# arthurlirui/IRON

Hardware: AMD Instinct MI355X
Metric: Mrays/s sphere-trace+GGX shade, drv/dragon 800x800 (synthetic S0) (higher is better)
Workload: dtype f32

## Files before the change

include/iron_hip.h:

```cpp
#ifndef IRON_HIP_H
#define IRON_HIP_H

#include <stddef.h>
#include <stdint.h>

#ifdef __cplusplus
extern "C" {
#endif

#define IRON_ABI_VERSION 1

typedef enum iron_status {
    IRON_OK = 0,
    IRON_ERR_BAD_ARG = -1,
    IRON_ERR_UNSUPPORTED = -2,
    IRON_ERR_HIP = -3,
    IRON_ERR_NO_DEVICE = -4,
    IRON_ERR_WORKSPACE = -5,
    IRON_ERR_RANGE = -6
} iron_status;

int iron_version(void);
const char* iron_strerror(int status);
int iron_last_hip_error(void);
// ... 245 lines not shown
                     const float* ray_d, const float* in0, const float* in1, const float* in2, const float* in3, const uint8_t* work,
                     int64_t n, uint8_t* mask_out, uint8_t* unfinished_out, float* points, float* sdf_out, float* dist,
                     void* workspace, size_t workspace_bytes, void* stream);

int iron_trace_phase(int32_t phase, const iron_net_t* sdf, const iron_trace_params* p, const float* lin_steps,
                     const float* ray_o, const float* ray_d, const float* near, const float* far,
                     const uint8_t* work, const int64_t* ray_index, int64_t n, int32_t* chunk_iters,
                     int64_t n_chunks, uint8_t* conv, float* points, float* sdf_out, float* dist,
                     iron_trace_stats* stats, void* workspace, size_t workspace_bytes, void* stream);

typedef struct iron_shade_nets {
    const iron_net_t* sdf;
    const iron_net_t* diffuse_albedo;
    const iron_net_t* specular_albedo;
    const iron_net_t* specular_roughness;
} iron_shade_nets;

typedef struct iron_shade_out {
    float* color;
    float* diffuse_color;
    float* specular_color;
    float* diffuse_albedo;
    float* specular_albedo;
    float* specular_roughness;
    float* normal;
} iron_shade_out;

size_t iron_shade_workspace_bytes(int64_t n);

int iron_shade_ggx(const iron_shade_nets* nets, float light, int32_t is_metal, const float* tab_trans,
                   const float* tab_diff_trans, const float* ray_o, const float* ray_d, const float* points,
                   const uint8_t* conv, int64_t n, const iron_shade_out* out, void* workspace,
                   size_t workspace_bytes, void* stream);

typedef struct iron_shade_comp_nets {
    const iron_net_t* sdf;
    const iron_net_t* diffuse_albedo;
    const iron_net_t* specular_albedo;
    const iron_net_t* specular_roughness;
    const iron_net_t* metallic;
    const iron_net_t* dielectric;
    const iron_net_t* metallic_eta;
    const iron_net_t* metallic_k;
    const iron_net_t* dielectric_eta;
} iron_shade_comp_nets;

typedef struct iron_shade_comp_out {
    float* color;
    float* diffuse_color;
    float* specular_color;
    float* diffuse_albedo;
    float* specular_albedo;
    float* specular_roughness;
    float* metallic_eta;
    float* metallic_k;
    float* dielectric_eta;
    float* normal;
    float* metallic_rgb;
    float* metallic;
    float* dielectric_rgb;
    float* dielectric;
} iron_shade_comp_out;

size_t iron_shade_composite_workspace_bytes(int64_t n);

int iron_shade_composite(const iron_shade_comp_nets* nets, float light, const float* tab_trans, const float* tab_diff_trans,
                         const float* ray_o, const float* ray_d, const float* points, const uint8_t* conv, int64_t n,
                         const iron_shade_comp_out* out, void* workspace, size_t workspace_bytes, void* stream);

int32_t iron_set_cu_limit(int32_t n_cus);

int32_t iron_set_trace_split(int32_t parts);

int iron_sdf_screen_forward(const iron_net_t* net, const float* x, int64_t n, float* out, void* stream);

int32_t iron_set_sampler_screen(int32_t on);
int iron_sampler_screen_debug(int32_t what, double value);
int iron_trace_screen_counts(const void* workspace, double* out, void* stream);

int32_t iron_set_sampler_stride(int32_t on);
int iron_trace_stride_counts(const void* workspace, double* out, void* stream);
int iron_trace_stride_detail(const void* workspace, double* out, void* stream);

enum {
    IRON_PROF_SPHERE = 0, IRON_PROF_SAMPLER = 1, IRON_PROF_BISECT_A = 2, IRON_PROF_BISECT_B = 3,
    IRON_PROF_SDF_GRAD = 4, IRON_PROF_MATERIAL = 5, IRON_PROF_GGX = 6, IRON_PROF_SDF_FORWARD = 7,
    IRON_PROF_KINDS = 8
};
int iron_profile_enable(int32_t on);
int iron_profile_read(double* ms, int64_t* launches);

#ifdef __cplusplus
}
#endif
#endif
```

iron_amd/_lib.py:

```python
from __future__ import annotations

import ctypes as C
import os
import threading
from typing import Optional

import torch

_HERE = os.path.dirname(os.path.abspath(__file__))
LIB_PATH = os.path.join(_HERE, "csrc", "libiron_hip.so")

IRON_OK = 0
IRON_NET_NERF = 2
IRON_ERR_UNSUPPORTED = -2
IRON_ERR_RANGE = -6
IRON_NET_SDF, IRON_NET_RENDER = 0, 1
MODES = {"idr": 0, "no_view_dir": 1, "no_normal": 2, "points_only": 3}


class IronError(RuntimeError):
    pass


class iron_linear(C.Structure):
# ... 83 lines not shown
    "iron_sdf_forward": (C.c_int, [_P, _P, _I64, _P, _I32, _P]),
    "iron_sdf_get_all_workspace_bytes": (_SZ, [_P, _I64]),
    "iron_sdf_get_all": (C.c_int, [_P, _P, _I64, _P, _P, _P, _P, _SZ, _P]),
    "iron_render_forward": (C.c_int, [_P, _P, _P, _P, _P, _I64, _P, _P]),
    "iron_camera_rays": (C.c_int, [C.POINTER(_F), C.POINTER(_F), _P, _I64, _P, _P, _P, _P]),
    "iron_intersect_sphere": (C.c_int, [_P, _P, _I64, _F, _P, _P, _P, _P]),
    "iron_ggx_colocated": (C.c_int, [_F, _P, _P, _P, _P, _P, _P, _P, _P, _I64, _P, _P, _P, _P]),
    "iron_composite_colocated": (C.c_int, [C.c_float, _P, _P, _P, _P, _P, _P, _I64, _P, _P, _P, _P, _P, _P]),
    "iron_coloc_head": (C.c_int, [_I32, C.c_float, C.c_float, C.c_float, _P, _P, _P, _P, _P, _P, _I64, _P, _P, _P, _P]),
    "iron_grid_points": (C.c_int, [_P, _P, _P, _I32, _I32, _I32, _P, _P]),
    "iron_mc_workspace_bytes": (C.c_int, [_I32, _I32, _I32, C.POINTER(_SZ)]),
    "iron_mc_count": (C.c_int, [_P, _I32, _I32, _I32, _F, _P, C.POINTER(_I64), C.POINTER(_I64), _P]),
    "iron_mc_emit": (C.c_int, [_P, _I32, _I32, _I32, _F, _P, _P, _P, _P]),
    "iron_bake_workspace_bytes": (C.c_int, [_I64, C.POINTER(_SZ)]),
    "iron_bake_count": (C.c_int, [_P, _I64, _P, _I64, _P, _I64, _I64, C.c_uint64, C.c_uint32, _P, _P, _P, C.POINTER(_I64), _P]),
    "iron_bake_sample": (C.c_int, [_P, _P, _P, _P, _I64, C.c_uint64, C.c_uint32, _P, _I64, _P, _P, _P, _P]),
    "iron_bake_sample_explicit": (C.c_int, [_P, _I64, _P, _P, _I64, _P, _I64, _P, _P, _P, _I64, _P, _P, _P]),
    "iron_bake_splat": (C.c_int, [_P, _P, _I32, _P, _I32, _I64, _I32, _I32, _I64, _P, _P, _P]),
    "iron_bake_resolve": (C.c_int, [_P, _I32, _I32, _I32, _P, _P, _P, _P]),
    "iron_bvh_workspace_bytes": (C.c_int, [_I64, C.POINTER(_SZ)]),
    "iron_bvh_keys": (C.c_int, [_P, _I64, _P, _I64, _P, _P, _P]),
    "iron_bvh_hierarchy": (C.c_int, [_P, _I64, _P, _P]),
    "iron_bvh_boxes": (C.c_int, [_P, _I64, _P, _I64, _P, _P, _P]),
    "iron_point_mesh_distance": (C.c_int, [_P, _I64, _P, _I64, _P, _P, _P, _P]),
    "iron_mesh_raycast": (C.c_int, [_P, _I64, _P, _P, _I64, _F, _F, _P, _P, _P, _P]),
    "iron_mesh_vertex_normals": (C.c_int, [_P, _I64, _P, _I64, _P, _P]),
    "iron_texture_fetch": (C.c_int, [_P, _P, _I32, _I32, _I32, _P, _I64, _I32, _P, _P, _P]),
    "iron_asset_shade_ggx": (C.c_int, [C.POINTER(iron_asset_mesh), _F, _P, _P, _P, _P, _P, _P, _P, _I64, C.POINTER(iron_asset_out), _P]),
    "iron_mesh_edge_keys": (C.c_int, [_P, _I64, _P, _I64, _P, _P, _P]),
    "iron_mesh_components": (C.c_int, [_P, _P, _I64, _P, _I64, _P, _P, _I32, C.POINTER(_I32), _P]),
    "iron_uv_workspace_bytes": (C.c_int, [_I64, C.POINTER(_SZ)]),
    "iron_uv_projections": (C.c_int, [_P, _I64, _P, _I64, _F, _F, _I32, _P, _P, _P, _P, _P, C.POINTER(_I32), C.POINTER(_I32), _P]),
    "iron_uv_project": (C.c_int, [_P, _P, _P, _I64, _P, _P, _P, _P]),
    "iron_uv_rotation_search": (C.c_int, [_P, _P, _I64, _I64, _P, _I32, _I32, _P, _P]),
    "iron_uv_apply": (C.c_int, [_P, _P, _I64, _P, _P, _F, _P, _P]),
    "iron_img_sqerr_workspace_bytes": (C.c_int, [_I64, C.POINTER(_SZ)]),
    "iron_img_sqerr": (C.c_int, [_P, _P, _I64, _I32, _P, _P, _P]),
    "iron_img_ssim_workspace_bytes": (C.c_int, [_I32, _I32, C.POINTER(_SZ)]),
    "iron_img_ssim": (C.c_int, [_P, _P, _I32, _I32, _I32, _P, _P, _P, _P]),
    "iron_lpips_prepare": (C.c_int, [_P, _P, _I32, _I32, _I32, _P, _P]),
    "iron_conv2d_relu": (C.c_int, [_P, _I32, _I32, _I32, _I32, _P, _P, _I32, _I32, _I32, _I32, _P, _P, _P]),
    "iron_maxpool3s2": (C.c_int, [_P, _I32, _I32, _I32, _I32, _P, _P]),
    "iron_lpips_tap": (C.c_int, [_P, _I32, _I32, _I32, _P, _P, _P]),
    "iron_lpips_workspace_bytes": (C.c_int, [_I32, _I32, C.POINTER(_SZ)]),
    "iron_lpips_forward": (C.c_int, [_P, _P, _I32, _I32, _I32, C.POINTER(iron_lpips_weights), _P, _P, _P]),
    "iron_neus_linspace": (C.c_int, [_P, _P, _P, _I64, _I32, _P, _P]),
    "iron_neus_outside_z": (C.c_int, [_P, _P, _I64, _I32, _F, _P, _P]),
    "iron_neus_points": (C.c_int, [_P, _P, _P, _I64, _I32, _P, _P]),
    "iron_neus_up_sample": (C.c_int, [_P, _P, _P, _P, _I64, _I32, _I32, _F, _P, _P]),
    "iron_neus_merge": (C.c_int, [_P, _P, _I32, _P, _P, _I32, _I64, _P, _P, _P]),
    "iron_neus_mid_points": (C.c_int, [_P, _P, _P, _I64, _I32, _F, _I32, _P, _P, _P, _P]),
    "iron_neus_need_background": (C.c_int, [_P, _I64, _I32, _I32, _P, _P]),
    "iron_neus_composite": (C.c_int, [C.POINTER(iron_neus_composite_args), _P]),
    "iron_neus_composite_alpha": (C.c_int, [C.POINTER(iron_neus_composite_args), _P, _P]),
    "iron_neus_outside_composite": (C.c_int, [_P, _P, _P, _P, _I64, _I32, _P, _P, _P, _P]),
    "iron_neus_sample_pdf": (C.c_int, [_P, _P, _P, _I64, _I32, _I32, _P, _P]),
    "iron_smith_g1": (C.c_int, [_P, _P, _I64, _P, _P]),
    "iron_nerf_forward": (C.c_int, [_P, _P, _P, _I64, _P, _P, _P]),
    "iron_edge_walk": (C.c_int, [_P, _P, _I64, _P, _I32, _F, _F, _P, _P, _P]),
    "iron_morph_closing3x3": (C.c_int, [_P, _I32, _I32, _P, _P, _P]),
    "iron_sobel_magnitude": (C.c_int, [_P, _I32, _I32, _P, _P]),
    "iron_edge_pixels": (C.c_int, [_P, _P, _I64, C.POINTER(_F), C.POINTER(_F), _I32, _I32, _P, _P, _P]),
    "iron_fill_holes": (C.c_int, [_P, _P, _P, _P, _I64, _P, _P, _P, _P, _P, _P]),
    "iron_edge_sides": (C.c_int, [_P, _P, C.POINTER(_F), _I64, _P, _P, _P]),
    "iron_edge_blend": (C.c_int, [_P, _P, _P, _P, _P, _P, _I64, _I64, _P, _P, _P, _P, _P]),
    "iron_trace_workspace_bytes": (_SZ, [_I64, C.POINTER(iron_trace_params)]),
    "iron_trace": (C.c_int, [_P, C.POINTER(iron_trace_params), _P, _P, _P, _P, _P, _P, _I64, _P, _P, _P, _P, _P,
                             _P, _SZ, _P]),
    "iron_trace_stage": (C.c_int, [_I32, _P, C.POINTER(iron_trace_params), _P, _P, _P, _P, _P, _P, _P, _P, _I64, _P, _P, _P, _P, _P,
                                   _P, _SZ, _P]),
    "iron_trace_phase": (C.c_int, [_I32, _P, C.POINTER(iron_trace_params), _P, _P, _P, _P, _P, _P, _P, _I64, _P,
                                   _I64, _P, _P, _P, _P, _P, _P, _SZ, _P]),
    "iron_net_numeric_status": (C.c_int, [_P, C.POINTER(C.c_int32), _P]),
    "iron_net_force_exact": (C.c_int, [_P, _I32]),
    "iron_set_cu_limit": (_I32, [_I32]),
    "iron_set_trace_split": (_I32, [_I32]),
    "iron_sdf_screen_forward": (C.c_int, [_P, _P, _I64, _P, _P]),
    "iron_set_sampler_screen": (_I32, [_I32]),
    "iron_sampler_screen_debug": (C.c_int, [_I32, C.c_double]),
    "iron_trace_screen_counts": (C.c_int, [_P, C.POINTER(C.c_double), _P]),
    "iron_set_sampler_stride": (_I32, [_I32]),
    "iron_trace_stride_counts": (C.c_int, [_P, C.POINTER(C.c_double), _P]),
    "iron_trace_stride_detail": (C.c_int, [_P, C.POINTER(C.c_double), _P]),
    "iron_profile_enable": (C.c_int, [_I32]),
    "iron_profile_read": (C.c_int, [C.POINTER(C.c_double), C.POINTER(_I64)]),
    "iron_shade_workspace_bytes": (_SZ, [_I64]),
    "iron_shade_composite_workspace_bytes": (_SZ, [_I64]),
    "iron_shade_composite": (C.c_int, [C.POINTER(iron_shade_comp_nets), _F, _P, _P, _P, _P, _P, _P, _I64,
                                       C.POINTER(iron_shade_comp_out), _P, _SZ, _P]),
    "iron_shade_ggx": (C.c_int, [C.POINTER(iron_shade_nets), _F, _I32, _P, _P, _P, _P, _P, _P, _I64,
                                 C.POINTER(iron_shade_out), _P, _SZ, _P]),
}

class iron_train_layer(C.Structure):
    _fields_ = [("weight_v", C.c_void_p), ("weight_g", C.c_void_p), ("bias", C.c_void_p), ("d_weight_v", C.c_void_p),
                ("d_weight_g", C.c_void_p), ("d_bias", C.c_void_p), ("out_dim", C.c_int32), ("in_dim", C.c_int32)]


class iron_sdf_train_desc(C.Structure):
    _fields_ = [("n_linear", C.c_int32), ("multires", C.c_int32), ("skip_layer", C.c_int32), ("layers", C.POINTER(iron_train_layer))]


class iron_render_train_desc(C.Structure):
    _fields_ = [("n_linear", C.c_int32), ("mode", C.c_int32), ("multires", C.c_int32), ("multires_view", C.c_int32),
                ("d_feature", C.c_int32), ("d_out", C.c_int32), ("skip_layer", C.c_int32), ("squeeze_out", C.c_int32),
                ("output_bias", C.c_float), ("output_scale", C.c_float), ("squeeze_out_scale", C.c_float),
                ("layers", C.POINTER(iron_train_layer))]


class iron_composite_grads_in(C.Structure):
    _fields_ = [(k, C.c_void_p) for k in ("d_rgb", "d_specular_rgb", "d_metallic_rgb", "d_dielectric_rgb", "d_env_light_out")]


class iron_composite_grads_out(C.Structure):
    _fields_ = [(k, C.c_void_p) for k in ("d_light", "d_distance", "d_normal", "d_viewdir", "d_diffuse_albedo", "d_specular_albedo",
                                          "d_specular_roughness", "d_metallic_eta", "d_metallic_k", "d_dielectric_eta", "d_env_light")]


class iron_nerf_train_desc(C.Structure):
    _fields_ = [("D", C.c_int32), ("W", C.c_int32), ("d_in", C.c_int32), ("d_in_view", C.c_int32), ("multires", C.c_int32),
                ("multires_view", C.c_int32), ("skip", C.c_int32), ("layers", C.POINTER(iron_train_layer))]


class iron_neus_composite_grads(C.Structure):
    _fields_ = [(k, C.c_void_p) for k in ("d_color", "d_weight_sum", "d_weights", "d_gradient_error", "relax_count", "d_sdf", "d_grad",
                                          "d_sample_color", "d_inv_s", "d_bg_density", "d_bg_color")]


TRAIN_LIB_PATH = os.path.join(os.path.dirname(LIB_PATH), "libiron_train.so")
TRAIN_SYMBOLS = {
    "iron_train_gemm_workspace_bytes": (_SZ, [_I32, _I32, _I32]),
    "iron_train_gemm": (C.c_int, [_I32, _I32, _I32, _I32, _I32, _P, _I32, _P, _I32, _F, _P, _I32, _P, _SZ, _P]),
    "iron_sdf_backward_workspace_bytes": (_SZ, [C.POINTER(iron_sdf_train_desc), _I64]),
    "iron_sdf_backward": (C.c_int, [C.POINTER(iron_sdf_train_desc), _P, _I64, _P, _P, _P, _P, _SZ, _P]),
    "iron_render_backward_workspace_bytes": (_SZ, [C.POINTER(iron_render_train_desc), _I64]),
    "iron_render_backward": (C.c_int, [C.POINTER(iron_render_train_desc), _P, _P, _P, _P, _I64, _P, _P, _P, _P, _P, _P, _SZ, _P]),
    "iron_ggx_colocated_backward": (C.c_int, [_F] + [_P] * 8 + [_I64] + [_P] * 10 + [_P]),
    "iron_composite_colocated_backward": (C.c_int, [_F, _P, _P, _P, C.POINTER(iron_composite_params), _P, _P, _I64,
                                                    C.POINTER(iron_composite_grads_in), C.POINTER(iron_composite_grads_out), _P]),
    "iron_coloc_head_backward": (C.c_int, [_I32, _F, _F, _F] + [_P] * 6 + [_I64] + [_P] * 10 + [_P]),
    "iron_nerf_backward_workspace_bytes": (_SZ, [C.POINTER(iron_nerf_train_desc), _I64]),
    "iron_nerf_backward": (C.c_int, [C.POINTER(iron_nerf_train_desc), _P, _P, _I64, _P, _P, _P, _SZ, _P]),
    "iron_neus_composite_backward": (C.c_int, [C.POINTER(iron_neus_composite_args), C.POINTER(iron_neus_composite_grads), _P]),
    "iron_train_last_hip_error": (C.c_int, []),
    "iron_train_last_blas_status": (C.c_int, []),
    "iron_train_numeric_status": (C.c_int, [_I32, _P]),
    "iron_pyramid_l2_workspace_bytes": (_SZ, [_I64, _I32, _I32]),
    "iron_pyramid_l2_forward": (C.c_int, [_P, _P, _I64, _I32, _I32, C.POINTER(C.c_float), _P, _P, _SZ, _P]),
    "iron_pyramid_l2_backward": (C.c_int, [_P, _P, _I64, _I32, _I32, C.POINTER(C.c_float), _P, _P, _SZ, _P, _P, _P]),
    "iron_ssim_workspace_bytes": (C.c_int, [_I32, _I32, _I32, _I32, _I32, _I32, C.POINTER(_SZ), C.POINTER(_SZ)]),
    "iron_ssim_forward": (C.c_int, [_P, _P, _I32, _I32, _I32, _I32, C.POINTER(C.c_float), _I32, C.c_double, C.c_double, _P, _I32, _P,
                                    _P, _SZ, _P]),
    "iron_ssim_backward": (C.c_int, [_P, _P, _I32, _I32, _I32, _I32, C.POINTER(C.c_float), _I32, C.c_double, C.c_double, _I32, _P, _P,
                                     _SZ, _P, _SZ, _P, _P, _P]),
    "iron_gaussian_filter": (C.c_int, [_P, _I64, _I32, _I32, C.POINTER(C.c_float), _I32, _P, _P]),
}

_lock = threading.Lock()
_lib: Optional[C.CDLL] = None
_train_lib: Optional[C.CDLL] = None


def load_train() -> C.CDLL:
    global _train_lib
    with _lock:
        if _train_lib is not None:
# ... 101 lines not shown
```

iron_amd/csrc/trace.hip:

```cpp
#include <atomic>
#include <mutex>
#include <stdlib.h>
#include "mlp_h2.h"
#include "ggx_core.h"
#include "h2_setup.h"

namespace iron {

constexpr int kMaxTraceSplits = 4;

#ifndef IRON_FAST_SOFTPLUS
#define IRON_FAST_SOFTPLUS 1
#endif
constexpr bool kFastActT = IRON_FAST_SOFTPLUS != 0;

struct SamplerQ {
    int n_list;
    int head;
    int n_cont;
    int n_done;
};

struct TraceCounters {
    int q_head;
// ... 80 lines not shown
constexpr int kResolvePerRay = 2;
constexpr uint8_t kRayPending = 2;
constexpr uint8_t kRayOverflowed = 1;
__device__ __forceinline__ float screen_delta(const ScreenWs& s) {
    return s.delta_override > 0.0f ? s.delta_override : fmaxf(kScreenK * __uint_as_float(*s.calib), kScreenFloor);
}

struct TraceWs {
    TraceCounters* cnt;
    int* sampler_list;
    int* root_list;
    float* root_lo;
    float* root_hi;
    float* root_flo;
    float* root_fhi;
    int* root_k;
    int* chunk_iters;
    int* chunk_roots;
    int n_chunks;
    unsigned long long* cont;
    int cont_cap;
    int ovf_pass;
    ScreenWs scr;
};

struct TraceArgs {
    const float* ray_o;
    const float* ray_d;
    const float* near;
    const float* far;
    const uint8_t* work;
    const int64_t* ray_index;
    const float* lin;
    uint8_t* conv;
    float* points;
    float* sdf;
    float* dist;
    int ray0;
    int n;
    int n_steps;
    int iters;
    float thr;
    long long chunk;
};

__device__ __forceinline__ int lane_rank(unsigned mask, int j) { return __popc(mask & ((1u << j) - 1u)); }
__device__ __forceinline__ int lane_rank64(unsigned long long mask, int j) { return __popcll(mask & ((1ull << j) - 1ull)); }

template <int HI = 32, int LO = 1, class T>
__device__ __forceinline__ T wave_sum(T x) {
#pragma unroll
    for (int off = HI; off >= LO; off >>= 1) x += __shfl_xor(x, off, 64);
    return x;
}
template <int HI = 32, int LO = 1>
__device__ __forceinline__ float wave_max(float x) {
#pragma unroll
    for (int off = HI; off >= LO; off >>= 1) x = fmaxf(x, __shfl_xor(x, off, 64));
    return x;
}

__device__ __forceinline__ void ray_origin_dir(const TraceArgs& a, int ray, float& ox, float& oy, float& oz, float& dx, float& dy, float& dz) {
    ox = a.ray_o[3 * (size_t)ray]; oy = a.ray_o[3 * (size_t)ray + 1]; oz = a.ray_o[3 * (size_t)ray + 2];
    dx = a.ray_d[3 * (size_t)ray]; dy = a.ray_d[3 * (size_t)ray + 1]; dz = a.ray_d[3 * (size_t)ray + 2];
}

struct BackendF32 {
    static constexpr int kThreads = 64;
    SdfNetDev net;
    WStream ws;
    int lane;
    __device__ __forceinline__ void init(const SdfNetDev& n, const H2StreamDev&, const H2Meta&) {
        net = n;
        lane = threadIdx.x;
        ws.init(net.blob, net.blob_bytes, lane);
    }
    __device__ __forceinline__ bool any(bool p) { return p; }
    __device__ __forceinline__ float eval(float x, float y, float z) { return sdf_eval<kFastActT>(net, ws, x, y, z, lane); }
    __device__ __forceinline__ void finish() {}
    __device__ __forceinline__ void park(int, float) {}
    __device__ __forceinline__ void park(int, int) {}
    __device__ __forceinline__ float unpark(int, float v) { return v; }
    __device__ __forceinline__ int unpark(int, int v) { return v; }
};

constexpr int kParkFields = 17;
constexpr int kLdsPark = kLdsH2Total;
constexpr int kLdsTraceTotal = kLdsPark + kParkFields * 256 * 4;
static_assert(kLdsTraceTotal <= 160 * 1024, "LDS of a tracer workgroup");

template <bool DEFER_TILES>
struct BackendH2T {
    static constexpr int kThreads = 256;
    Ring ring;
    char* lds;
    H2Meta m;
    int lane, wave, parity;
    __device__ __forceinline__ void init(const SdfNetDev&, const H2StreamDev& s, const H2Meta& meta) {
        extern __shared__ __attribute__((aligned(16))) char smem[];
        lds = smem;
        m = meta;
        lane = threadIdx.x & 63;
        wave = __builtin_amdgcn_readfirstlane(threadIdx.x >> 6);
        parity = 0;
        h2_setup(s, lds, ring);
    }
    __device__ __forceinline__ bool any(bool p) {
        volatile int* f = reinterpret_cast<volatile int*>(lds + kLdsMisc) + parity * 4;
        if (lane == 0) f[wave] = p ? 1 : 0;
        __syncthreads();
        const int r = f[0] | f[1] | f[2] | f[3];
        parity ^= 1;
        return r != 0;
    }
    __device__ __forceinline__ float eval(float x, float y, float z) {
        f32x16 hf[kHidTiles];
        sdf_hidden_stack_h2<kFastActT, DEFER_TILES>(ring, lds, m.n_hidden_layers, m.skip_layer, m.scale, x, y, z, lane, hf);
        return (row_dot_lds(lds + kLdsRows, hf, lane >> 5) + m.b_last) / m.scale;
    }
    template <int NP>
    __device__ __forceinline__ float eval_screen(float x, float y, float z) {
        return sdf_screen_value<kFastActT, NP>(ring, lds, m.n_hidden_layers, m.skip_layer, m.scale, m.b_last, x, y, z, lane);
    }
    __device__ __forceinline__ void finish() { ring.drain(); }
    __device__ __forceinline__ void park(int i, float v) { reinterpret_cast<float*>(lds + kLdsPark)[i * 256 + threadIdx.x] = v; }
    __device__ __forceinline__ void park(int i, int v) { reinterpret_cast<int*>(lds + kLdsPark)[i * 256 + threadIdx.x] = v; }
    __device__ __forceinline__ float unpark(int i, float) { return reinterpret_cast<const float*>(lds + kLdsPark)[i * 256 + threadIdx.x]; }
    __device__ __forceinline__ int unpark(int i, int) { return reinterpret_cast<const int*>(lds + kLdsPark)[i * 256 + threadIdx.x]; }
};

#ifndef IRON_TRACE_DEFER
#define IRON_TRACE_DEFER 1
#endif
typedef BackendH2T<IRON_TRACE_DEFER != 0> BackendH2;
#ifndef IRON_SAMPLER_DEFER
#define IRON_SAMPLER_DEFER 1
#endif
typedef BackendH2T<IRON_SAMPLER_DEFER != 0> BackendH2Sampler;

template <class BE>
__device__ __forceinline__ void park_i64(BE& be, int i, long long v) { be.park(i, (int)(unsigned)v); be.park(i + 1, (int)(v >> 32)); }
template <class BE>
__device__ __forceinline__ long long unpark_i64(BE& be, int i, long long v) {
    return (long long)(((unsigned long long)(unsigned)be.unpark(i + 1, (int)(v >> 32)) << 32) | (unsigned)be.unpark(i, (int)(unsigned)v));
}
template <class BE>
__device__ __forceinline__ void park_vec6(BE& be, int i, float ox, float oy, float oz, float dx, float dy, float dz) {
    be.park(i, ox); be.park(i + 1, oy); be.park(i + 2, oz); be.park(i + 3, dx); be.park(i + 4, dy); be.park(i + 5, dz);
}
template <class BE>
__device__ __forceinline__ void unpark_vec6(BE& be, int i, float& ox, float& oy, float& oz, float& dx, float& dy, float& dz) {
    ox = be.unpark(i, ox); oy = be.unpark(i + 1, oy); oz = be.unpark(i + 2, oz);
    dx = be.unpark(i + 3, dx); dy = be.unpark(i + 4, dy); dz = be.unpark(i + 5, dz);
}

#define IRON_TRACE_KERNEL_ARGS SdfNetDev net, H2StreamDev hs, H2Meta hm, TraceArgs a, TraceWs w

template <class BE>
__global__ __launch_bounds__(BE::kThreads, 1) void k_sphere(IRON_TRACE_KERNEL_ARGS) {
    BE be;
    be.init(net, hs, hm);
    const int lane = be.lane;
    const int j = lane & 31;

    bool active = false, unf = false, work = false, exhausted = false;
    int ray = 0, steps = 0;
    float px = 0.f, py = 0.f, pz = 0.f, dx = 0.f, dy = 0.f, dz = 0.f, t = 0.f, far = 0.f;
    long long evals = 0, nconv = 0;

    for (;;) {
        const unsigned act = (unsigned)__ballot(active);
        const int nfree = 32 - __popc(act);
        if (nfree > 0 && !exhausted) {
            int base = 0;
            if (lane == 0) base = atomicAdd(&w.cnt->q_head, nfree);
            base = __shfl(base, 0, 64);
            int avail = a.n - base;
            avail = avail < 0 ? 0 : (avail > nfree ? nfree : avail);
            if (base + nfree >= a.n) exhausted = true;
            const int rank = lane_rank(~act, j);
            if (!active && rank < avail) {
                ray = a.ray0 + base + rank;
                const float ox = a.ray_o[3 * (size_t)ray], oy = a.ray_o[3 * (size_t)ray + 1], oz = a.ray_o[3 * (size_t)ray + 2];
                dx = a.ray_d[3 * (size_t)ray]; dy = a.ray_d[3 * (size_t)ray + 1]; dz = a.ray_d[3 * (size_t)ray + 2];
                t = a.near[ray];
                far = a.far[ray];
                work = a.work[ray] != 0;
                unf = work;
                px = ox + dx * t; py = oy + dy * t; pz = oz + dz * t;
                steps = 0;
                active = true;
            }
        }
        const unsigned act2 = (unsigned)__ballot(active);
        if (!be.any(act2 != 0u)) break;
        evals += __popc(act2);

        {
            const int flags = (active ? 1 : 0) | (unf ? 2 : 0) | (work ? 4 : 0) | (exhausted ? 8 : 0);
            be.park(0, flags); be.park(1, ray); be.park(2, steps);
            be.park(3, px); be.park(4, py); be.park(5, pz); be.park(6, dx); be.park(7, dy); be.park(8, dz); be.park(9, t); be.park(10, far);
            be.park(11, (int)(unsigned)evals); be.park(12, (int)(evals >> 32)); be.park(13, (int)(unsigned)nconv); be.park(14, (int)(nconv >> 32));
        }
        const float s = be.eval(px, py, pz);
        {
            const int flags = be.unpark(0, (active ? 1 : 0) | (unf ? 2 : 0) | (work ? 4 : 0) | (exhausted ? 8 : 0));
            active = flags & 1; unf = flags & 2; work = flags & 4; exhausted = flags & 8;
            ray = be.unpark(1, ray); steps = be.unpark(2, steps);
            px = be.unpark(3, px); py = be.unpark(4, py); pz = be.unpark(5, pz); dx = be.unpark(6, dx); dy = be.unpark(7, dy); dz = be.unpark(8, dz);
            t = be.unpark(9, t); far = be.unpark(10, far);
            evals = (long long)(((unsigned long long)(unsigned)be.unpark(12, (int)(evals >> 32)) << 32) | (unsigned)be.unpark(11, (int)(unsigned)evals));
            nconv = (long long)(((unsigned long long)(unsigned)be.unpark(14, (int)(nconv >> 32)) << 32) | (unsigned)be.unpark(13, (int)(unsigned)nconv));
        }

        bool retire = false, to_sampler = false;
        if (active) {
            unf = unf && (fabsf(s) > a.thr) && (t < far);
            if (!unf || steps == a.iters) {
                retire = true;
                to_sampler = unf;
            } else {
                t += s;
                px += dx * s; py += dy * s; pz += dz * s;
                ++steps;
            }
        }
        const unsigned samp = (unsigned)__ballot(to_sampler);
        int sbase = 0;
        if (samp) {
            if (lane == 0) sbase = atomicAdd(&w.cnt->smp.n_list, __popc(samp));
            sbase = __shfl(sbase, 0, 64);
        }
        if (retire) {
            if (lane < 32) {
                const bool conv = work && !unf && (fabsf(s) <= a.thr) && (t < far);
                a.conv[ray] = conv ? 1 : 0;
                a.points[3 * (size_t)ray] = px; a.points[3 * (size_t)ray + 1] = py; a.points[3 * (size_t)ray + 2] = pz;
                a.sdf[ray] = s;
                a.dist[ray] = t;
                if (to_sampler) w.sampler_list[sbase + lane_rank(samp, j)] = ray;
                if (conv) ++nconv;
            }
            active = false;
            px = py = pz = 0.f;
        }
    }
    be.finish();
    long long c = nconv;
#pragma unroll
    for (int off = 32; off > 0; off >>= 1) c += __shfl_xor(c, off, 64);
    if (lane == 0) {
        atomicAdd((unsigned long long*)&w.cnt->n_evals, (unsigned long long)evals);
        atomicAdd((unsigned long long*)&w.cnt->n_evals_sphere, (unsigned long long)evals);
        atomicAdd((unsigned long long*)&w.cnt->n_sphere_conv, (unsigned long long)c);
    }
}

#ifndef IRON_SAMPLER_BLOCK
#define IRON_SAMPLER_BLOCK 8
#endif
#ifndef IRON_SAMPLER_SEG
#define IRON_SAMPLER_SEG 4
#endif
constexpr int kSamplerBlock = IRON_SAMPLER_BLOCK;
constexpr int kSamplerSlots = 32 / kSamplerBlock;
constexpr int kScreenSlots = 32 * kH1PointTiles / kSamplerBlock;
static_assert(kScreenSlots <= 32, "screen slots: one bit each in a 32-bit slot mask");
constexpr int kSamplerSeg = IRON_SAMPLER_SEG;
static_assert(kSamplerBlock == 4 || kSamplerBlock == 8 || kSamplerBlock == 16 || kSamplerBlock == 32, "sampler block");
constexpr int kContRayBits = 24, kContBlkBits = 8;

static inline int64_t sampler_cont_cap(int64_t n, int n_steps) {
    if (kSamplerSeg <= 0) return 0;
    const int64_t blocks = (n_steps + kSamplerBlock - 1) / kSamplerBlock;
    if (n + 2 >= (1ll << kContRayBits) || blocks >= (1ll << kContBlkBits)) return 0;
    const int64_t segs = (blocks + kSamplerSeg - 1) / kSamplerSeg;
    if (n * (segs - 1) * 8 > (256ll << 20)) return 0;
    return n * (segs - 1);
}

__device__ __forceinline__ float sample_depth(float smin, float lin, float width) { return smin + lin * width; }


template <int SLOTS, class Ballot>
__device__ __forceinline__ unsigned slot_heads(Ballot b) {
    unsigned m = 0;
#pragma unroll
    for (int s = 0; s < SLOTS; ++s) m |= (unsigned)((b >> (s * kSamplerBlock)) & (Ballot)1) << s;
    return m;
}
// ... 788 lines not shown
        out->n_sphere_conv = n_sphere_conv;
        out->n_sampler = n_sampler;
        out->n_bisect = n_root;
        out->n_conv = n_sphere_conv + n_root;
        long long e = n_evals_sphere + n_sampler * n_steps;
        for (int c = 0; c < w.n_chunks; ++c) e += (long long)w.chunk_roots[c] * (w.chunk_iters[c] + 1);
        out->n_evals_ref = e;
        out->n_evals_sphere = n_evals_sphere;
        out->reserved = n_abort;
    }
}

__global__ void k_stage_mark_list(const int* __restrict__ list, const int* __restrict__ count, uint8_t* __restrict__ mask) {
    const int n = *count;
    for (int i = blockIdx.x * blockDim.x + threadIdx.x; i < n; i += gridDim.x * blockDim.x) mask[list[i]] = 1;
}

__global__ void k_stage_sampler_init(TraceArgs a, TraceWs w, const float* __restrict__ min_dis) {
    for (int i = blockIdx.x * blockDim.x + threadIdx.x; i < a.n; i += gridDim.x * blockDim.x) {
        w.sampler_list[i] = i;
        a.dist[i] = min_dis[i];
        a.sdf[i] = 1.0f;
    }
    if (blockIdx.x == 0 && threadIdx.x == 0) w.cnt->smp.n_list = a.n;
}

__global__ void k_stage_root_init(TraceWs w, int n, const float* __restrict__ f_low, const float* __restrict__ f_high,
                                  const float* __restrict__ d_low, const float* __restrict__ d_high) {
    for (int i = blockIdx.x * blockDim.x + threadIdx.x; i < n; i += gridDim.x * blockDim.x) {
        w.root_list[i] = i;
        w.root_lo[i] = d_low[i]; w.root_hi[i] = d_high[i];
        w.root_flo[i] = f_low[i]; w.root_fhi[i] = f_high[i];
    }
    if (blockIdx.x == 0 && threadIdx.x == 0) w.cnt->n_root = n;
}

static inline size_t align256(size_t x) { return (x + 255) & ~(size_t)255; }

struct WsLayout {
    size_t cnt, sampler_list, root_list, lo, hi, flo, fhi, k, chunk_iters, chunk_roots, cont, total;
    size_t s_rec, s_pend, s_ovf, s_flag, s_ent;
    int64_t n_chunks, cont_cap;
};

static WsLayout ws_layout(int64_t n, const iron_trace_params* p) {
    WsLayout L;
    const size_t nn = (size_t)(n > 0 ? n : 1);
    L.n_chunks = (p && p->chunk > 0) ? (n + p->chunk - 1) / p->chunk : 1;
    if (L.n_chunks < 1) L.n_chunks = 1;
    size_t o = 0;
    static_assert(sizeof(TraceCounters) <= kCntStride, "counter block");
    L.cnt = o; o += kCntStride * kMaxTraceSplits;
    L.chunk_iters = o; o += align256(sizeof(int) * (size_t)L.n_chunks);
    L.chunk_roots = o; o += align256(sizeof(int) * (size_t)L.n_chunks);
    L.sampler_list = o; o += align256(sizeof(int) * nn);
    L.root_list = o; o += align256(sizeof(int) * nn);
    L.lo = o; o += align256(sizeof(float) * nn);
    L.hi = o; o += align256(sizeof(float) * nn);
    L.flo = o; o += align256(sizeof(float) * nn);
    L.fhi = o; o += align256(sizeof(float) * nn);
    L.k = o; o += align256(sizeof(int) * nn);
    L.cont_cap = sampler_cont_cap(n, p ? p->n_steps : 128);
    L.cont = o; o += align256(sizeof(unsigned long long) * (size_t)(L.cont_cap > 0 ? L.cont_cap : 1));
    L.s_rec = o; o += align256(sizeof(PendRec) * nn);
    L.s_pend = o; o += align256(sizeof(int) * nn);
    L.s_ovf = o; o += align256(sizeof(int) * nn);
    L.s_flag = o; o += align256(nn);
    L.s_ent = o; o += align256(sizeof(ResolveEntry) * nn * kResolvePerRay);
    L.total = o;
    return L;
}

static int resident_waves() {
    return cu_budget() * 4;
}

enum TraceKernel { kSphere = 0, kSampler = 1, kBisectA = 2, kBisectB = 3, kSamplerScreen = 4, kScreenResolve = 5, kScreenCalib = 6 };

static void launch_trace_kernel(TraceKernel which, bool h2, const iron_net* sdf, const TraceArgs& a, const TraceWs& w, int64_t units,
                                hipStream_t st) {
    H2Meta m;
    m.n_hidden_layers = sdf->sdf.n_hidden_layers; m.skip_layer = sdf->sdf.skip_layer; m.scale = sdf->sdf.scale; m.b_last = sdf->sdf.b_last;
    if (units < 1) units = 1;
    if (h2) {
        static bool attr = false;
        if (!attr) {
            const void* const kernels[] = {(const void*)k_sphere<BackendH2>, (const void*)k_sampler<BackendH2Sampler>, (const void*)k_bisect_a<BackendH2>,
                                           (const void*)k_bisect_b<BackendH2>, (const void*)k_sampler_screen<BackendH2Sampler>,
                                           (const void*)k_screen_resolve<BackendH2>, (const void*)k_screen_calib};
            for (const void* k : kernels) (void)hipFuncSetAttribute(k, hipFuncAttributeMaxDynamicSharedMemorySize, kLdsTraceTotal);
            attr = true;
        }
        const int64_t wgs = (units + 3) / 4;
        const int cus = resident_waves() / 4;
        const dim3 grid((unsigned)(wgs < cus ? wgs : cus)), block(256);
        switch (which) {
            case kSphere: hipLaunchKernelGGL(k_sphere<BackendH2>, grid, block, kLdsTraceTotal, st, sdf->sdf, sdf->h2_trace, m, a, w); break;
            case kSampler: hipLaunchKernelGGL(k_sampler<BackendH2Sampler>, grid, block, kLdsTraceTotal, st, sdf->sdf, sdf->h2_trace, m, a, w); break;
            case kBisectA: hipLaunchKernelGGL(k_bisect_a<BackendH2>, grid, block, kLdsTraceTotal, st, sdf->sdf, sdf->h2_trace, m, a, w); break;
            case kSamplerScreen: hipLaunchKernelGGL(k_sampler_screen<BackendH2Sampler>, grid, block, kLdsTraceTotal, st, sdf->sdf, sdf->h1_trace, m, a, w); break;
            case kScreenResolve: hipLaunchKernelGGL(k_screen_resolve<BackendH2>, grid, block, kLdsTraceTotal, st, sdf->sdf, sdf->h2_trace, m, a, w); break;
            case kScreenCalib: hipLaunchKernelGGL(k_screen_calib, dim3(cus < kScreenCalibPoints / 128 ? cus : kScreenCalibPoints / 128), block,
                                                  kLdsTraceTotal, st, sdf->sdf, sdf->h2_trace, sdf->h1_trace, m, sdf->screen_calib); break;
            default: hipLaunchKernelGGL(k_bisect_b<BackendH2>, grid, block, kLdsTraceTotal, st, sdf->sdf, sdf->h2_trace, m, a, w); break;
        }
    } else {
        const int waves = resident_waves();
        const dim3 grid((unsigned)(units < waves ? units : waves)), block(64);
        switch (which) {
            case kSphere: hipLaunchKernelGGL(k_sphere<BackendF32>, grid, block, 0, st, sdf->sdf, sdf->h2_trace, m, a, w); break;
            case kSampler: hipLaunchKernelGGL(k_sampler<BackendF32>, grid, block, 0, st, sdf->sdf, sdf->h2_trace, m, a, w); break;
            case kBisectA: hipLaunchKernelGGL(k_bisect_a<BackendF32>, grid, block, 0, st, sdf->sdf, sdf->h2_trace, m, a, w); break;
            default: hipLaunchKernelGGL(k_bisect_b<BackendF32>, grid, block, 0, st, sdf->sdf, sdf->h2_trace, m, a, w); break;
        }
    }
}

std::atomic<int> g_screen_switch{-1};
std::atomic<float> g_screen_delta_override{0.0f};
std::atomic<int> g_screen_cap_override{0};
std::atomic<int> g_stride_switch{-1};
std::atomic<float> g_stride_l_override{0.0f};
std::atomic<int> g_stride_hooks{0};
void set_screen_forward_tiles(int point_tiles);

static bool env_switch(const char* name, const std::atomic<int>& set, int* from_env) {
    if (*from_env < 0) {
        const char* e = getenv(name);
        *from_env = (e && e[0] == '0') ? 0 : 1;
    }
    const int v = set.load(std::memory_order_relaxed);
    return v < 0 ? *from_env != 0 : v != 0;
}
static bool screen_switch() { static int from_env = -1; return env_switch("IRON_SAMPLER_SCREEN", g_screen_switch, &from_env); }
static bool stride_switch() { static int from_env = -1; return env_switch("IRON_SAMPLER_STRIDE", g_stride_switch, &from_env); }

static int screen_begin(const iron_net* cnet, bool h2, hipStream_t st, bool* use) {
    iron_net* net = const_cast<iron_net*>(cnet);
    *use = false;
    if (net->flag_host && *(volatile int*)(net->flag_host + 1)) net->screen_off = 1;
    if (net->flag_host && *(volatile int*)(net->flag_host + 2)) net->stride_off = 1;
    if (!h2 || !screen_switch() || net->screen_off || !net->h1_trace.base) return IRON_OK;
    if (!net->screen_calib) IRON_HIP_TRY(hipMalloc((void**)&net->screen_calib, kScreenCalibBytes));
    if (!net->screen_calibrated) {
        IRON_HIP_TRY(hipMemsetAsync(net->screen_calib, 0, 256, st));
        TraceArgs a{};
        TraceWs w{};
        launch_trace_kernel(kScreenCalib, true, net, a, w, kScreenCalibPoints / 32, st);
        net->screen_calibrated = 1;
    }
    *use = true;
    return IRON_OK;
}

static void screen_ws(TraceWs& w, const iron_net* net, char* base, const WsLayout& L, int64_t b0, int64_t nk, int n_steps) {
    w.scr.calib = net->screen_calib;
    w.scr.stride = (stride_switch() && !net->stride_off && n_steps <= kStrideMaxSteps && w.cont_cap > 0)
                       ? (kStrideOn | g_stride_hooks.load(std::memory_order_relaxed)) : 0;
    w.scr.l_override = g_stride_l_override.load(std::memory_order_relaxed);
    w.scr.flag = net->flag_dev ? net->flag_dev + 1 : nullptr;
    w.scr.delta_override = g_screen_delta_override.load(std::memory_order_relaxed);
    w.scr.rec = (PendRec*)(base + L.s_rec);
    w.scr.ray_state = (uint8_t*)(base + L.s_flag);
    w.scr.pend_list = (int*)(base + L.s_pend) + b0;
    w.scr.ovf_list = (int*)(base + L.s_ovf) + b0;
    w.scr.ent = (ResolveEntry*)(base + L.s_ent) + b0 * kResolvePerRay;
// ... 45 lines not shown
    w.chunk_roots = (int*)(base + L.chunk_roots);
    w.n_chunks = (int)L.n_chunks;
    w.cont = (unsigned long long*)(base + L.cont);
    w.cont_cap = (int)L.cont_cap;
    return w;
}

}

using namespace iron;

static int32_t set_switch(std::atomic<int>& set, bool prev, int32_t on) {
    set.store(on < 0 ? -1 : (on ? 1 : 0), std::memory_order_relaxed);
    return prev ? 1 : 0;
}
extern "C" int32_t iron_set_sampler_screen(int32_t on) { return set_switch(g_screen_switch, screen_switch(), on); }
extern "C" int32_t iron_set_sampler_stride(int32_t on) { return set_switch(g_stride_switch, stride_switch(), on); }

extern "C" int iron_sampler_screen_debug(int32_t what, double value) {
    if (what == 0) { g_screen_delta_override.store(value > 0.0 ? (float)value : 0.0f, std::memory_order_relaxed); return IRON_OK; }
    if (what == 1) { g_screen_cap_override.store(value >= 1.0 ? (int)value : 0, std::memory_order_relaxed); return IRON_OK; }
    if (what == 2) { set_screen_forward_tiles(value == 1.0 ? 1 : 0); return IRON_OK; }
    if (what == 3) { g_stride_l_override.store(value > 0.0 ? (float)value : 0.0f, std::memory_order_relaxed); return IRON_OK; }
    if (what == 4 || what == 5) {
        const int bit = what == 4 ? kStridePendingOff : kStrideMuteMarch;
        if (value != 0.0) g_stride_hooks.fetch_or(bit, std::memory_order_relaxed);
        else g_stride_hooks.fetch_and(~bit, std::memory_order_relaxed);
        return IRON_OK;
    }
    return IRON_ERR_BAD_ARG;
}

static int read_counters(const void* workspace, hipStream_t stream, TraceCounters out[kMaxTraceSplits]) {
    for (int k = 0; k < kMaxTraceSplits; ++k)
        IRON_HIP_TRY(hipMemcpyAsync(&out[k], (const char*)workspace + (size_t)k * kCntStride, sizeof(TraceCounters), hipMemcpyDeviceToHost, stream));
    IRON_HIP_TRY(hipStreamSynchronize(stream));
    return IRON_OK;
}
static void max_f32_bits(double* m, unsigned bits) {
    const float r = __builtin_bit_cast(float, bits);
    if (r > *m) *m = r;
}

extern "C" int iron_trace_screen_counts(const void* workspace, double* out, void* stream) {
    if (!workspace || !out) return IRON_ERR_BAD_ARG;
    TraceCounters c[kMaxTraceSplits];
    const int rc = read_counters(workspace, (hipStream_t)stream, c);
    if (rc != IRON_OK) return rc;
    double scr = 0, res = 0, ovf = 0, ratio = 0, pend = 0;
    for (int k = 0; k < kMaxTraceSplits; ++k) {
        scr += (double)c[k].n_screen; res += (double)c[k].n_resolved; ovf += (double)c[k].n_ovf; pend += (double)c[k].n_pend;
        max_f32_bits(&ratio, c[k].ratio_bits);
    }
    out[0] = scr; out[1] = res; out[2] = ovf; out[3] = ratio; out[4] = pend;
    return IRON_OK;
}

extern "C" int iron_trace_stride_counts(const void* workspace, double* out, void* stream) {
    if (!workspace || !out) return IRON_ERR_BAD_ARG;
    TraceCounters c[kMaxTraceSplits];
    const int rc = read_counters(workspace, (hipStream_t)stream, c);
    if (rc != IRON_OK) return rc;
    double passes = 0, strided = 0, ratio = 0, mode = 0;
    for (int k = 0; k < kMaxTraceSplits; ++k) {
        passes += (double)c[k].n_pass; strided += (double)c[k].n_pass_strided;
        max_f32_bits(&ratio, c[k].slope_bits);
        if (c[k].stride_mode) mode = 1;
    }
    out[0] = passes; out[1] = strided; out[2] = ratio; out[3] = mode;
    return IRON_OK;
}

extern "C" int iron_trace_stride_detail(const void* workspace, double* out, void* stream) {
    if (!workspace || !out) return IRON_ERR_BAD_ARG;
    TraceCounters c[kMaxTraceSplits];
    const int rc = read_counters(workspace, (hipStream_t)stream, c);
    if (rc != IRON_OK) return rc;
    for (int i = 0; i < 9; ++i) out[i] = 0.0;
    for (int k = 0; k < kMaxTraceSplits; ++k) {
        out[0] += (double)c[k].n_pass_behind; out[1] += (double)c[k].n_pass_fresh; out[2] += (double)c[k].n_restart;
        out[3] += (double)c[k].n_obs_march; out[4] += (double)c[k].n_obs_res; out[5] += (double)c[k].n_obs_pair;
        max_f32_bits(&out[6], c[k].slope_march_bits); max_f32_bits(&out[7], c[k].slope_res_bits); max_f32_bits(&out[8], c[k].slope_pair_bits);
    }
    return IRON_OK;
}

extern "C" size_t iron_trace_workspace_bytes(int64_t n, const iron_trace_params* p) {
    if (n < 0) return 0;
    return ws_layout(n, p).total + align256(sizeof(int) * 65536);
}

namespace iron {
namespace {
struct SideStreams {
    bool ready = false;
    hipStream_t s[kMaxTraceSplits - 1];
    hipEvent_t fork, join[kMaxTraceSplits - 1];
};
std::mutex g_side_mu;
SideStreams g_side[64];

std::atomic<int> g_trace_split{0};
int trace_splits(int64_t n) {
    static int from_env = -1;
    if (from_env < 0) {
        const char* e = getenv("IRON_TRACE_SPLIT");
        from_env = e ? atoi(e) : 0;
        if (from_env < 0) from_env = 0;
    }
    int k = g_trace_split.load(std::memory_order_relaxed);
    if (k <= 0) k = from_env;
    if (k < 1) k = 1;
    if (k > kMaxTraceSplits) k = kMaxTraceSplits;
    while (k > 1 && n < (int64_t)k * 256) --k;
    return k;
}

int side_streams(SideStreams** out) {
    int dev = 0;
    IRON_HIP_TRY(hipGetDevice(&dev));
    if (dev < 0 || dev >= 64) return IRON_ERR_UNSUPPORTED;
    SideStreams& S = g_side[dev];
    if (!S.ready) {
        int least = 0, greatest = 0;
        IRON_HIP_TRY(hipDeviceGetStreamPriorityRange(&least, &greatest));
        for (int i = 0; i < kMaxTraceSplits - 1; ++i) {
            IRON_HIP_TRY(hipStreamCreateWithPriority(&S.s[i], hipStreamNonBlocking, least));
            IRON_HIP_TRY(hipEventCreateWithFlags(&S.join[i], hipEventDisableTiming));
        }
        IRON_HIP_TRY(hipEventCreateWithFlags(&S.fork, hipEventDisableTiming));
        S.ready = true;
    }
    *out = &S;
    return IRON_OK;
}
}
}

extern "C" int32_t iron_set_trace_split(int32_t parts) {
    return g_trace_split.exchange(parts > 0 ? (parts > kMaxTraceSplits ? kMaxTraceSplits : parts) : 0, std::memory_order_relaxed);
}

extern "C" int iron_trace_phase(int32_t phase, const iron_net_t* sdf, const iron_trace_params* p, const float* lin_steps,
                                const float* ray_o, const float* ray_d, const float* near, const float* far,
                                const uint8_t* work, const int64_t* ray_index, int64_t n, int32_t* chunk_iters,
                                int64_t n_chunks, uint8_t* conv, float* points, float* sdf_out, float* dist,
                                iron_trace_stats* stats, void* workspace, size_t workspace_bytes, void* stream) {
    if (phase != 0 && phase != 1) return IRON_ERR_BAD_ARG;
    const bool args_ok = lin_steps && ray_o && ray_d && near && far && work && conv && points && sdf_out && dist;
    WsLayout L;
    const int rcc = check_trace_call(sdf, p, n, args_ok, p ? p->chunk : 0, workspace, workspace_bytes, &L);
    if (rcc != IRON_OK || n == 0) return rcc;
    if (chunk_iters && (n_chunks < 1 || n_chunks > 65536)) return IRON_ERR_BAD_ARG;
    hipStream_t st = (hipStream_t)stream;
    char* base = (char*)workspace;
    TraceWs w0 = bind_workspace(base, L);
    if (chunk_iters) { w0.chunk_iters = chunk_iters; w0.n_chunks = (int)n_chunks; }
    if (chunk_iters && n_chunks > L.n_chunks) {
        if (workspace_bytes < L.total + align256(sizeof(int) * (size_t)n_chunks)) return IRON_ERR_WORKSPACE;
        w0.chunk_roots = (int*)(base + L.total);
    }
    TraceArgs a0;
    a0.ray_o = ray_o; a0.ray_d = ray_d; a0.near = near; a0.far = far; a0.work = work; a0.ray_index = ray_index;
    a0.lin = lin_steps; a0.conv = conv; a0.points = points; a0.sdf = sdf_out; a0.dist = dist;
    a0.ray0 = 0; a0.n = (int)n; a0.n_steps = p->n_steps; a0.iters = p->sphere_tracing_iters; a0.thr = p->sdf_threshold;
    a0.chunk = p->chunk > 0 ? p->chunk : 0;
// ... 131 lines not shown
```

Baseline: 18.08.

## Batch sphere-trace ray claims into per-wave stock and prefetch ray data via LDS DMA

In the sphere-tracing kernel, each wave now claims a stock of 64 rays per atomic instead of exactly the number of free slots. Near the end of the queue the claim size tapers with the rays left, to keep load balanced across waves. After each claim, the wave issues one LDS DMA per lane over the cache lines of the claimed rays' origin, direction, near/far and work entries, so later loads hit in cache. This cuts contention on the global counter and hides ray-fetch latency, at the cost of more parked state, a little more LDS, and coarser work distribution. It also adds optional static-assignment and prewarm modes, both off by default, and a counter-readout API.

New measurement: 17.87. -1.2%, worse.

```diff
diff --git a/include/iron_hip.h b/include/iron_hip.h
--- a/include/iron_hip.h
+++ b/include/iron_hip.h
@@ -351,6 +351,8 @@
 int iron_trace_stride_counts(const void* workspace, double* out, void* stream);
 int iron_trace_stride_detail(const void* workspace, double* out, void* stream);
 
+int iron_trace_sphere_counts(const void* workspace, double* out, void* stream);
+
 enum {
     IRON_PROF_SPHERE = 0, IRON_PROF_SAMPLER = 1, IRON_PROF_BISECT_A = 2, IRON_PROF_BISECT_B = 3,
     IRON_PROF_SDF_GRAD = 4, IRON_PROF_MATERIAL = 5, IRON_PROF_GGX = 6, IRON_PROF_SDF_FORWARD = 7,
diff --git a/iron_amd/_lib.py b/iron_amd/_lib.py
--- a/iron_amd/_lib.py
+++ b/iron_amd/_lib.py
@@ -189,6 +189,7 @@
     "iron_set_sampler_stride": (_I32, [_I32]),
     "iron_trace_stride_counts": (C.c_int, [_P, C.POINTER(C.c_double), _P]),
     "iron_trace_stride_detail": (C.c_int, [_P, C.POINTER(C.c_double), _P]),
+    "iron_trace_sphere_counts": (C.c_int, [_P, C.POINTER(C.c_double), _P]),
     "iron_profile_enable": (C.c_int, [_I32]),
     "iron_profile_read": (C.c_int, [C.POINTER(C.c_double), C.POINTER(_I64)]),
     "iron_shade_workspace_bytes": (_SZ, [_I64]),
diff --git a/iron_amd/csrc/trace.hip b/iron_amd/csrc/trace.hip
--- a/iron_amd/csrc/trace.hip
+++ b/iron_amd/csrc/trace.hip
@@ -186,11 +186,13 @@
     __device__ __forceinline__ void park(int, int) {}
     __device__ __forceinline__ float unpark(int, float v) { return v; }
     __device__ __forceinline__ int unpark(int, int v) { return v; }
+    __device__ __forceinline__ void touch(const char*, bool) {}
 };
 
 constexpr int kParkFields = 17;
 constexpr int kLdsPark = kLdsH2Total;
-constexpr int kLdsTraceTotal = kLdsPark + kParkFields * 256 * 4;
+constexpr int kLdsTouch = kLdsPark + kParkFields * 256 * 4;
+constexpr int kLdsTraceTotal = kLdsTouch + 4 * 256;
 static_assert(kLdsTraceTotal <= 160 * 1024, "LDS of a tracer workgroup");
 
 template <bool DEFER_TILES>
@@ -231,6 +233,11 @@
     __device__ __forceinline__ void park(int i, int v) { reinterpret_cast<int*>(lds + kLdsPark)[i * 256 + threadIdx.x] = v; }
     __device__ __forceinline__ float unpark(int i, float) { return reinterpret_cast<const float*>(lds + kLdsPark)[i * 256 + threadIdx.x]; }
     __device__ __forceinline__ int unpark(int i, int) { return reinterpret_cast<const int*>(lds + kLdsPark)[i * 256 + threadIdx.x]; }
+    __device__ __forceinline__ void touch(const char* p, bool on) {
+        int wv = wave;
+        asm volatile("" : "+s"(wv));
+        if (on) lds_dma4(p, lds_addr_of(lds + kLdsTouch) + (uint32_t)wv * 256u);
+    }
 };
 
 #ifndef IRON_TRACE_DEFER
@@ -260,6 +267,55 @@
 
 #define IRON_TRACE_KERNEL_ARGS SdfNetDev net, H2StreamDev hs, H2Meta hm, TraceArgs a, TraceWs w
 
+#ifndef IRON_SPHERE_STOCK
+#define IRON_SPHERE_STOCK 64
+#endif
+#ifndef IRON_SPHERE_TOUCH
+#define IRON_SPHERE_TOUCH 1
+#endif
+#ifndef IRON_SPHERE_STATIC
+#define IRON_SPHERE_STATIC 0
+#endif
+#ifndef IRON_SPHERE_PREWARM
+#define IRON_SPHERE_PREWARM 0
+#endif
+#ifndef IRON_SPHERE_TAPER
+#define IRON_SPHERE_TAPER 1
+#endif
+constexpr bool kSphereTaper = IRON_SPHERE_TAPER != 0;
+constexpr bool kSphereStatic = IRON_SPHERE_STATIC != 0;
+constexpr int kSphereStock = kSphereStatic ? 32 : IRON_SPHERE_STOCK;
+constexpr bool kSphereTouch = IRON_SPHERE_TOUCH != 0 && kSphereStock > 0;
+static_assert(kSphereStock == 0 || (kSphereStock >= 32 && kSphereStock <= 128), "a draw must cover one pass's free slots; touch: one line per lane");
+
+template <class BE>
+__device__ __forceinline__ void sphere_touch_stock(BE& be, const TraceArgs& a, int lane, unsigned d, unsigned e) {
+    constexpr int kL3 = (kSphereStock * 12 + 127) / 128 + 1, kL1 = (kSphereStock * 4 + 127) / 128 + 1, kL0 = (kSphereStock + 127) / 128 + 1;
+    static_assert(2 * kL3 + 2 * kL1 + kL0 <= 64, "one line per lane");
+    asm volatile("" : "+v"(lane));
+    int i = lane;
+    const char* p = reinterpret_cast<const char*>(a.ray_o);
+    size_t stride = 12;
+    if (i >= kL3) { i -= kL3; p = reinterpret_cast<const char*>(a.ray_d); }
+    if (lane >= 2 * kL3) { i -= kL3; p = reinterpret_cast<const char*>(a.near); stride = 4; }
+    if (lane >= 2 * kL3 + kL1) { i -= kL1; p = reinterpret_cast<const char*>(a.far); }
+    if (lane >= 2 * kL3 + 2 * kL1) { i -= kL1; p = reinterpret_cast<const char*>(a.work); stride = 1; }
+    const uintptr_t first = (uintptr_t)p + ((size_t)a.ray0 + d) * stride, end = (uintptr_t)p + ((size_t)a.ray0 + e) * stride;
+    uintptr_t q = (first & ~(uintptr_t)127) + 128u * (unsigned)i;
+    if (q < first) q = (first + 3) & ~(uintptr_t)3;
+    be.touch(reinterpret_cast<const char*>(q), lane < 2 * kL3 + 2 * kL1 + kL0 && q + 4 <= end);
+}
+
+__global__ void k_sphere_prewarm(TraceArgs a, int* sink) {
+    const size_t n = (size_t)a.n, r0 = (size_t)a.ray0;
+    unsigned acc = 0;
+    for (size_t i = blockIdx.x * (size_t)blockDim.x + threadIdx.x; i < 3 * n; i += (size_t)gridDim.x * blockDim.x) {
+        acc ^= __float_as_uint(a.ray_o[3 * r0 + i]) ^ __float_as_uint(a.ray_d[3 * r0 + i]);
+        if (i < n) acc ^= __float_as_uint(a.near[r0 + i]) ^ __float_as_uint(a.far[r0 + i]) ^ a.work[r0 + i];
+    }
+    if (a.n < 0) *sink = (int)acc;
+}
+
 template <class BE>
 __global__ __launch_bounds__(BE::kThreads, 1) void k_sphere(IRON_TRACE_KERNEL_ARGS) {
     BE be;
@@ -271,20 +327,60 @@
     int ray = 0, steps = 0;
     float px = 0.f, py = 0.f, pz = 0.f, dx = 0.f, dy = 0.f, dz = 0.f, t = 0.f, far = 0.f;
     long long evals = 0, nconv = 0;
+    unsigned s_next = 0u, s_end = 0u;
+    if constexpr (kSphereStatic) s_next = s_end = 32u * (blockIdx.x * (BE::kThreads / 64) + (threadIdx.x >> 6));
 
     for (;;) {
         const unsigned act = (unsigned)__ballot(active);
         const int nfree = 32 - __popc(act);
-        if (nfree > 0 && !exhausted) {
-            int base = 0;
-            if (lane == 0) base = atomicAdd(&w.cnt->q_head, nfree);
-            base = __shfl(base, 0, 64);
-            int avail = a.n - base;
-            avail = avail < 0 ? 0 : (avail > nfree ? nfree : avail);
-            if (base + nfree >= a.n) exhausted = true;
+        if (nfree > 0 && (kSphereStock > 0 || !exhausted)) {
             const int rank = lane_rank(~act, j);
-            if (!active && rank < avail) {
-                ray = a.ray0 + base + rank;
+            unsigned ticket = 0;
+            bool got = false;
+            if constexpr (kSphereStock == 0) {
+                int base = 0;
+                if (lane == 0) base = atomicAdd(&w.cnt->q_head, nfree);
+                base = __shfl(base, 0, 64);
+                if (base + nfree >= a.n) exhausted = true;
+                ticket = (unsigned)(base + rank);
+                got = ticket < (unsigned)a.n;
+            } else {
+                const unsigned have = s_end - s_next;
+                ticket = s_next + (unsigned)rank;
+                got = (unsigned)rank < have;
+                if (have < (unsigned)nfree && !exhausted) {
+                    const unsigned need = (unsigned)nfree - have;
+                    unsigned take = (unsigned)kSphereStock, d;
+                    if constexpr (kSphereStatic) {
+                        const unsigned g32 = 32u * (blockIdx.x * (BE::kThreads / 64) + (threadIdx.x >> 6)), stride = 32u * gridDim.x * (BE::kThreads / 64);
+                        d = s_end == g32 ? g32 : s_end - 32u + stride;
+                        exhausted = d + stride >= (unsigned)a.n;
+                    } else {
+                        if constexpr (kSphereTaper) {
+                            const unsigned left = ((unsigned)a.n - s_end) >> (31 - __clz((int)(gridDim.x * (BE::kThreads / 64))));
+                            take = left < take ? (left > need ? left : need) : take;
+                        }
+                        int b = 0;
+                        if (lane == 0) b = (int)atomicAdd(reinterpret_cast<unsigned*>(&w.cnt->q_head), take);
+                        d = (unsigned)__builtin_amdgcn_readfirstlane(b);
+                        exhausted = d + take >= (unsigned)a.n;
+                    }
+                    d = d < (unsigned)a.n ? d : (unsigned)a.n;
+                    s_end = d + take < (unsigned)a.n ? d + take : (unsigned)a.n;
+                    if (!got) {
+                        ticket = d + ((unsigned)rank - have);
+                        got = ticket < s_end;
+                    }
+                    s_next = d + need < s_end ? d + need : s_end;
+                    if constexpr (kSphereTouch) {
+                        if (d < s_end) sphere_touch_stock(be, a, lane, d, s_end);
+                    }
+                } else {
+                    s_next += have < (unsigned)nfree ? have : (unsigned)nfree;
+                }
+            }
+            if (!active && got) {
+                ray = a.ray0 + (int)ticket;
                 const float ox = a.ray_o[3 * (size_t)ray], oy = a.ray_o[3 * (size_t)ray + 1], oz = a.ray_o[3 * (size_t)ray + 2];
                 dx = a.ray_d[3 * (size_t)ray]; dy = a.ray_d[3 * (size_t)ray + 1]; dz = a.ray_d[3 * (size_t)ray + 2];
                 t = a.near[ray];
@@ -305,11 +401,13 @@
             be.park(0, flags); be.park(1, ray); be.park(2, steps);
             be.park(3, px); be.park(4, py); be.park(5, pz); be.park(6, dx); be.park(7, dy); be.park(8, dz); be.park(9, t); be.park(10, far);
             be.park(11, (int)(unsigned)evals); be.park(12, (int)(evals >> 32)); be.park(13, (int)(unsigned)nconv); be.park(14, (int)(nconv >> 32));
+            be.park(15, (int)s_next); be.park(16, (int)s_end);
         }
         const float s = be.eval(px, py, pz);
         {
             const int flags = be.unpark(0, (active ? 1 : 0) | (unf ? 2 : 0) | (work ? 4 : 0) | (exhausted ? 8 : 0));
             active = flags & 1; unf = flags & 2; work = flags & 4; exhausted = flags & 8;
+            s_next = (unsigned)__builtin_amdgcn_readfirstlane(be.unpark(15, (int)s_next)); s_end = (unsigned)__builtin_amdgcn_readfirstlane(be.unpark(16, (int)s_end));
             ray = be.unpark(1, ray); steps = be.unpark(2, steps);
             px = be.unpark(3, px); py = be.unpark(4, py); pz = be.unpark(5, pz); dx = be.unpark(6, dx); dy = be.unpark(7, dy); dz = be.unpark(8, dz);
             t = be.unpark(9, t); far = be.unpark(10, far);
@@ -1264,6 +1362,8 @@
     H2Meta m;
     m.n_hidden_layers = sdf->sdf.n_hidden_layers; m.skip_layer = sdf->sdf.skip_layer; m.scale = sdf->sdf.scale; m.b_last = sdf->sdf.b_last;
     if (units < 1) units = 1;
+    if (IRON_SPHERE_PREWARM != 0 && which == kSphere)
+        hipLaunchKernelGGL(k_sphere_prewarm, dim3(1024), dim3(256), 0, st, a, &w.cnt->q_head);
     if (h2) {
         static bool attr = false;
         if (!attr) {
@@ -1475,6 +1575,19 @@
         out[3] += (double)c[k].n_obs_march; out[4] += (double)c[k].n_obs_res; out[5] += (double)c[k].n_obs_pair;
         max_f32_bits(&out[6], c[k].slope_march_bits); max_f32_bits(&out[7], c[k].slope_res_bits); max_f32_bits(&out[8], c[k].slope_pair_bits);
     }
+    return IRON_OK;
+}
+
+extern "C" int iron_trace_sphere_counts(const void* workspace, double* out, void* stream) {
+    if (!workspace || !out) return IRON_ERR_BAD_ARG;
+    TraceCounters c[kMaxTraceSplits];
+    const int rc = read_counters(workspace, (hipStream_t)stream, c);
+    if (rc != IRON_OK) return rc;
+    out[0] = out[1] = out[2] = 0.0;
+    for (int k = 0; k < kMaxTraceSplits; ++k) {
+        out[0] += (double)c[k].n_evals_sphere; out[1] += (double)c[k].n_sphere_conv; out[2] += (double)c[k].smp.n_list;
+    }
+    out[3] = (double)kSphereStock;
     return IRON_OK;
 }
 
```
